# seceq/zkir

Hardware: AMD Instinct MI355X
Metric: trace rows/sec (2^20-cycle fib: execution-trace fill + BabyBear NTT/LDE + Poseidon2 Merkle commitment) (higher is better)
Workload: dtype u32 (Baby Bear, 31-bit modular) / u64 trace words

## Files before the change

zkir_amd/csrc/ntt.hip:

```cpp
#include <hip/hip_runtime.h>

#include <atomic>
#include <cstdlib>
#include <mutex>
#include <type_traits>

#include "../../include/zkir_amd.h"
#include "../../include/zkir_amd_experimental.h"
#include "babybear.h"
#include "host.h"

namespace {

constexpr int NT = 256;
__device__ __forceinline__ uint32_t bitrev(uint32_t x, int bits) { return bits == 0 ? 0u : __brev(x) >> (32 - bits); }

template <int K, int N, class F>
__device__ __forceinline__ void static_for(F&& f) {
  if constexpr (K < N) { f(std::integral_constant<int, K>{}); static_for<K + 1, N>(f); }
}

using u32x4 = uint32_t __attribute__((ext_vector_type(4)));
__device__ __forceinline__ u32x4 ld4(const uint4* p) { return *reinterpret_cast<const u32x4*>(p); }
__device__ __forceinline__ void st4(uint4* p, u32x4 v) { *reinterpret_cast<u32x4*>(p) = v; }

__device__ __forceinline__ void wave_sync_lds() { asm volatile("s_waitcnt lgkmcnt(0)" ::: "memory"); }

struct WTw { int32_t w, n; };
__device__ __forceinline__ WTw wtw(int32_t w) { return WTw{w, -w}; }
__device__ __forceinline__ void dit4w4(uint4& x0, uint4& x1, uint4& x2, uint4& x3, WTw w1, WTw w2, WTw w2i) {
#define ZKIR_Q(c, e) { int32_t a[4] = {(int32_t)x0.c, (int32_t)x1.c, (int32_t)x2.c, (int32_t)x3.c}, b[4] = {(int32_t)x0.e, (int32_t)x1.e, (int32_t)x2.e, (int32_t)x3.e}; \
                       bb::dit4w2(a, b, w1.w, w1.n, w2.w, w2.n, w2i.w, w2i.n); \
                       x0.c = (uint32_t)a[0]; x1.c = (uint32_t)a[1]; x2.c = (uint32_t)a[2]; x3.c = (uint32_t)a[3]; x0.e = (uint32_t)b[0]; x1.e = (uint32_t)b[1]; x2.e = (uint32_t)b[2]; x3.e = (uint32_t)b[3]; }
  ZKIR_Q(x, y) __builtin_amdgcn_sched_barrier(0); ZKIR_Q(z, w)
#undef ZKIR_Q
}
__device__ __forceinline__ void ct4w4(uint4& x0, uint4& x1, uint4& x2, uint4& x3, WTw w1, WTw w2, WTw w2i) { dit4w4(x0, x2, x1, x3, w1, w2, w2i); }
__device__ __forceinline__ void ct_twiddles(uint32_t sm, uint32_t f, bool unit, uint32_t j4_m, WTw& w1, WTw& w2, WTw& w2i) {
  uint32_t w2u;
  if (unit) { w2u = sm; w2 = wtw(bb::centre(sm)); }
  else { w2 = wtw(bb::mont_mul_centred(sm, f)); w2u = bb::wcanon(w2.w); }
  w1 = wtw(bb::mont_mul_centred(w2u, w2u)); w2i = wtw(bb::mont_mul_centred(w2u, j4_m));
}
__device__ __forceinline__ uint4 scale4(uint4 v, uint32_t g) {
  int32_t x[4] = {(int32_t)v.x, (int32_t)v.y, (int32_t)v.z, (int32_t)v.w};
  bb::wscale4(x, g);
  return make_uint4((uint32_t)x[0], (uint32_t)x[1], (uint32_t)x[2], (uint32_t)x[3]);
}
__device__ __forceinline__ void dit2w4(uint4& a, uint4& b, WTw w) {
#define ZKIR_Q(c) { int32_t p = (int32_t)a.c, q = (int32_t)b.c; bb::dit2w(p, q, w.w, w.n); a.c = (uint32_t)p; b.c = (uint32_t)q; }
  ZKIR_Q(x) ZKIR_Q(y) ZKIR_Q(z) ZKIR_Q(w)
#undef ZKIR_Q
}
__device__ __forceinline__ uint4 canon4(uint4 v) { return make_uint4(bb::wcanon((int32_t)v.x), bb::wcanon((int32_t)v.y), bb::wcanon((int32_t)v.z), bb::wcanon((int32_t)v.w)); }

template <bool DIT>
__global__ __launch_bounds__(NT) void ntt_stage_kernel(uint4* __restrict__ data, uint64_t blk_u4, int L, int s0, const uint32_t* __restrict__ tw, int canon) {
  uint4* x = data + (uint64_t)blockIdx.y * blk_u4;
  const uint64_t item = (uint64_t)blockIdx.x * NT + threadIdx.x;
  const uint32_t n = 1u << L;
  if (item >= (uint64_t)n) return;
  const uint32_t t = (uint32_t)(item >> 1), h = (uint32_t)(item & 1);
  uint32_t p, stride, w;
  if (DIT) { stride = 1u << s0; const uint32_t hi = t >> s0, lo = t & (stride - 1); p = (hi << (s0 + 1)) + lo; w = tw[lo << (L - s0 - 1)]; }
  else { stride = n >> (s0 + 1); const uint32_t hi = t / stride, lo = t % stride; p = hi * (n >> s0) + lo; w = tw[bitrev(hi, s0) << (L - s0 - 1)]; }
  uint4 a = x[(uint64_t)p * 2 + h], b = x[(uint64_t)(p + stride) * 2 + h];
  dit2w4(a, b, wtw(bb::centre(w)));
  if (DIT && canon) { a = canon4(a); b = canon4(b); }
  x[(uint64_t)p * 2 + h] = a; x[(uint64_t)(p + stride) * 2 + h] = b;
}

struct TraceSrc01 { zkir_trace_columns t; uint64_t n_real; };
__device__ __forceinline__ u32x4 trace_quad01(const TraceSrc01& q, uint32_t blk, uint32_t half, uint64_t i) {
  const bool pad = i >= q.n_real;
  const uint64_t src = pad ? q.n_real - 1 : i;
  u32x4 r;
  if (blk == 0 && half == 0) {
    const uint64_t pcv = q.t.pc[src];
    r.x = (uint32_t)((q.t.cycle[src] + (i - src)) % bb::P); r.y = (uint32_t)(pcv & 0xFFFFF); r.z = (uint32_t)((pcv >> 20) & 0xFFFFF); r.w = (uint32_t)(pcv >> 40);
  } else if (blk == 0) {
    const uint32_t w = q.t.instruction[src];
    r.x = w & 0x7F; r.y = (w >> 7) & 0xF; r.z = (w >> 11) & 0xF; r.w = (w >> 15) & 0xF;
  } else {
    auto limbs = [&](int g, uint32_t out[3]) {
      const uint64_t o = (uint64_t)g * q.t.reg_stride + src;
      const uint64_t v = q.t.registers[o];
      const int bits = q.t.reg_state[o] ? 30 : 20;
      const uint64_t mask = (1ull << bits) - 1;
      out[0] = (uint32_t)(v & mask); out[1] = (uint32_t)((v >> bits) & mask); out[2] = (uint32_t)(v >> (2 * bits));
    };
    uint32_t a[3], b[3];
    if (half == 0) { limbs(1, a); r.x = q.t.instruction[src] >> 19; r.y = a[0]; r.z = a[1]; r.w = a[2]; }
    else { limbs(2, a); limbs(3, b); r.x = a[0]; r.y = a[1]; r.z = a[2]; r.w = b[0]; }
  }
  return r;
}

template <bool DIT, int R, int C, int NTH, bool FUSED = false>
__global__ __launch_bounds__(NTH) void ntt_strided_r4_kernel(uint4* __restrict__ data, uint64_t blk_u4, uint32_t tiles_per_block, uint32_t total, int L, int s0,
                                                              const uint32_t* __restrict__ tw, const uint32_t* __restrict__ small, int log_small, uint32_t j4_m, int canon, TraceSrc01 fsrc = TraceSrc01{}) {
  constexpr int B = 2 * R;
  constexpr uint32_t POS = 1u << (B + C), QUADS = POS / 4, CMASK = (1u << C) - 1, PLANE = POS + 4;
  constexpr uint32_t MOVES = 2 * POS / NTH;
  static_assert(QUADS % NTH == 0 && NTH % (1 << C) == 0 && (2 * POS) % NTH == 0, "tile / thread geometry");
  extern __shared__ uint4 lds4[];
  const uint32_t n = 1u << L;
  const uint32_t stride_mid = DIT ? (1u << s0) : (n >> (s0 + B));
  const uint32_t lo_tiles = stride_mid >> C;
  auto geometry = [&](uint32_t w, uint4*& x, uint32_t& base, uint32_t& lo0, uint32_t& hi) {
    const uint32_t tile = w % tiles_per_block;
    x = data + (uint64_t)(w / tiles_per_block) * blk_u4;
    hi = tile / lo_tiles;
    lo0 = (tile % lo_tiles) << C;
    base = (DIT ? (hi << (s0 + B)) : hi * (n >> s0)) + lo0;
  };
  static_assert(QUADS == NTH, "one quad per lane and round");
  u32x4 pre[MOVES];
  uint4* x; uint32_t base, lo0, hi;
  uint32_t w = blockIdx.x;
  if (w >= total) return;
  uint32_t sm[R];
#pragma unroll
  for (int r = 0; r < R; r++) {
    const int b = 2 * r;
    const uint32_t qq = threadIdx.x >> C;
    if (!DIT) sm[r] = small[bitrev(qq >> (B - 2 - b), b) << (log_small - (b + 2))];
    else sm[r] = small[(qq & ((1u << b) - 1)) << (log_small - (b + 2))];
  }
  const bool unit = s0 == 0;
  uint32_t tf_next[R] = {};
  auto tile_factors = [&](uint32_t hi_t) {
    if (DIT || unit) return;
    const uint32_t e = bitrev(hi_t, s0);
#pragma unroll
    for (int r = 0; r < R; r++) tf_next[r] = tw[e << (L - s0 - 2 * r - 2)];
  };
  geometry(w, x, base, lo0, hi);
  static_for<0, (int)MOVES>([&](auto kc) {
    constexpr uint32_t k = decltype(kc)::value;
    const uint32_t e = threadIdx.x + k * NTH, row = e >> (C + 1), wv = e & ((2u << C) - 1);
    if constexpr (FUSED) pre[k] = trace_quad01(fsrc, w / tiles_per_block, wv & 1, (uint64_t)base + (uint64_t)row * stride_mid + (wv >> 1));
    else pre[k] = ld4(&x[((uint64_t)base + (uint64_t)row * stride_mid) * 2 + wv]);
  });
  uint32_t tw_cur = 0;
  if (DIT) tw_cur = tw[(lo0 + (threadIdx.x & CMASK)) << (L - s0 - B)];
  tile_factors(hi);
  for (;;) {
    static_for<0, (int)MOVES>([&](auto kc) {
      constexpr uint32_t k = decltype(kc)::value;
      const uint32_t e = threadIdx.x + k * NTH, row = e >> (C + 1), wv = e & ((2u << C) - 1);
      st4(&lds4[(wv & 1) * PLANE + ((row << C) | (wv >> 1))], pre[k]);
    });
    uint32_t tp[R];
    if (DIT) {
      uint32_t u = tw_cur;
#pragma unroll
      for (int r = R - 1; r >= 0; r--) { tp[r] = u; u = bb::mont_mul(u, u); u = bb::mont_mul(u, u); }
    } else {
#pragma unroll
      for (int r = 0; r < R; r++) tp[r] = tf_next[r];
    }
    __syncthreads();
    const uint32_t wn = w + gridDim.x;
    uint4* xn = x; uint32_t base_n = base, lo0_n = lo0, hi_n = hi;
    if (wn < total) {
      geometry(wn, xn, base_n, lo0_n, hi_n);
      static_for<0, (int)MOVES>([&](auto kc) {
        constexpr uint32_t k = decltype(kc)::value;
        const uint32_t e = threadIdx.x + k * NTH, row = e >> (C + 1), wv = e & ((2u << C) - 1);
        if constexpr (FUSED) pre[k] = trace_quad01(fsrc, wn / tiles_per_block, wv & 1, (uint64_t)base_n + (uint64_t)row * stride_mid + (wv >> 1));
        else pre[k] = ld4(&xn[((uint64_t)base_n + (uint64_t)row * stride_mid) * 2 + wv]);
      });
      if (DIT) tw_cur = tw[(lo0_n + (threadIdx.x & CMASK)) << (L - s0 - B)];
      tile_factors(hi_n);
    }
#pragma unroll
    for (int r = 0; r < R; r++) {
      const int b = 2 * r;
#pragma unroll
      for (uint32_t k = 0; k < QUADS / NTH; k++) {
        uint32_t q = threadIdx.x + k * NTH;
        asm volatile("" : "+v"(q));
        const uint32_t lo_l = q & CMASK, qq = q >> C;
        uint4* pl0 = lds4; uint4* pl1 = lds4 + PLANE;
        if constexpr (!DIT) {
          const int lg = B - 2 - b;
          const uint32_t h2 = 1u << lg, mid_lo = qq & (h2 - 1), mid_hi = qq >> lg;
          const uint32_t i0 = ((((mid_hi << (lg + 2)) | mid_lo)) << C) | lo_l, d = h2 << C;
          WTw w1, w2, w2i;
          ct_twiddles(sm[r], tp[r], unit, j4_m, w1, w2, w2i);
          uint4 x0 = pl0[i0], x1 = pl0[i0 + d], x2 = pl0[i0 + 2 * d], x3 = pl0[i0 + 3 * d];
          ct4w4(x0, x1, x2, x3, w1, w2, w2i);
          pl0[i0] = x0; pl0[i0 + d] = x1; pl0[i0 + 2 * d] = x2; pl0[i0 + 3 * d] = x3;
          __builtin_amdgcn_sched_barrier(0);
          uint4 y0 = pl1[i0], y1 = pl1[i0 + d], y2 = pl1[i0 + 2 * d], y3 = pl1[i0 + 3 * d];
          ct4w4(y0, y1, y2, y3, w1, w2, w2i);
          pl1[i0] = y0; pl1[i0 + d] = y1; pl1[i0 + 2 * d] = y2; pl1[i0 + 3 * d] = y3;
        } else {
          const uint32_t dm = 1u << b, mid_lo = qq & (dm - 1), mid_hi = qq >> b;
          const uint32_t i0 = ((((mid_hi << (b + 2)) | mid_lo)) << C) | lo_l, d = dm << C;
          const WTw w2 = wtw(bb::mont_mul_centred(tp[r], sm[r]));
          const uint32_t w2u = bb::wcanon(w2.w);
          const WTw w1 = wtw(bb::mont_mul_centred(w2u, w2u)), w2i = wtw(bb::mont_mul_centred(w2u, j4_m));
          uint4 x0 = pl0[i0], x1 = pl0[i0 + d], x2 = pl0[i0 + 2 * d], x3 = pl0[i0 + 3 * d];
          dit4w4(x0, x1, x2, x3, w1, w2, w2i);
          pl0[i0] = x0; pl0[i0 + d] = x1; pl0[i0 + 2 * d] = x2; pl0[i0 + 3 * d] = x3;
          __builtin_amdgcn_sched_barrier(0);
          uint4 y0 = pl1[i0], y1 = pl1[i0 + d], y2 = pl1[i0 + 2 * d], y3 = pl1[i0 + 3 * d];
          dit4w4(y0, y1, y2, y3, w1, w2, w2i);
          pl1[i0] = y0; pl1[i0 + d] = y1; pl1[i0 + 2 * d] = y2; pl1[i0 + 3 * d] = y3;
        }
      }
      const bool wave_local = !DIT ? (r + 1 < R && B - 2 - b <= 6 - C) : (r + 1 < R && b + 2 <= 6 - C);
      if (wave_local) wave_sync_lds(); else __syncthreads();
    }
#pragma unroll
    for (uint32_t k = 0; k < MOVES; k++) {
      const uint32_t e = threadIdx.x + k * NTH, row = e >> (C + 1), wv = e & ((2u << C) - 1);
      uint4 v = lds4[(wv & 1) * PLANE + ((row << C) | (wv >> 1))];
      if (DIT && canon) v = canon4(v);
      x[((uint64_t)base + (uint64_t)row * stride_mid) * 2 + wv] = v;
    }
    if (wn >= total) break;
    w = wn; x = xn; base = base_n; lo0 = lo0_n; hi = hi_n;
  }
}

template <bool DIT, int S>
__global__ __launch_bounds__(NT) void ntt_reg_kernel(uint4* __restrict__ data, uint64_t blk_u4, int L, int s0, const uint32_t* __restrict__ tw, uint32_t r4_m, uint32_t r8_m,
                                                       uint32_t r8_3_m, int canon) {
  constexpr int E = 1 << S;
  const uint32_t n = 1u << L;
  uint4* x = data + (uint64_t)blockIdx.y * blk_u4;
  const uint64_t item = (uint64_t)blockIdx.x * NT + threadIdx.x;
  if (item >= ((uint64_t)n >> S) * 2) return;
  const uint32_t t = (uint32_t)(item >> 1), h = (uint32_t)(item & 1);
  const uint32_t d = DIT ? (1u << s0) : (n >> (s0 + S));
  const uint32_t hi = t / d, lo = t % d;
  const uint64_t base = ((uint64_t)hi * d * E + lo) * 2 + h;
  uint4 v[E];
#pragma unroll
  for (int k = 0; k < E; k++) v[k] = x[base + (uint64_t)k * d * 2];
  if (!DIT) {
    const uint32_t Tf = tw[bitrev(hi, s0) << (L - s0 - S)];
    const uint32_t Tm = bb::mont_mul(Tf, Tf);
    if (S == 3) {
      const WTw t0 = wtw(bb::mont_mul_centred(Tm, Tm)), tm = wtw(bb::centre(Tm)), m1 = wtw(bb::mont_mul_centred(Tm, r4_m));
#pragma unroll
      for (int g = 0; g < 2; g++) ct4w4(v[g], v[g + 2], v[g + 4], v[g + 6], t0, tm, m1);
      const WTw wf[4] = {wtw(bb::centre(Tf)), wtw(bb::mont_mul_centred(Tf, r4_m)), wtw(bb::mont_mul_centred(Tf, r8_m)), wtw(bb::mont_mul_centred(Tf, r8_3_m))};
#pragma unroll
      for (int m = 0; m < 4; m++) dit2w4(v[2 * m], v[2 * m + 1], wf[m]);
    } else {
      ct4w4(v[0], v[1], v[2], v[3], wtw(bb::centre(Tm)), wtw(bb::centre(Tf)), wtw(bb::mont_mul_centred(Tf, r4_m)));
    }
  } else {
    const uint32_t Uf = tw[lo << (L - s0 - S)];
    const uint32_t Um = bb::mont_mul(Uf, Uf);
    if (S == 3) {
      const WTw u0 = wtw(bb::mont_mul_centred(Um, Um)), um = wtw(bb::centre(Um)), m1 = wtw(bb::mont_mul_centred(Um, r4_m));
#pragma unroll
      for (int g = 0; g < 8; g += 4) dit4w4(v[g], v[g + 1], v[g + 2], v[g + 3], u0, um, m1);
      const WTw wf[4] = {wtw(bb::centre(Uf)), wtw(bb::mont_mul_centred(Uf, r8_m)), wtw(bb::mont_mul_centred(Uf, r4_m)), wtw(bb::mont_mul_centred(Uf, r8_3_m))};
#pragma unroll
      for (int k = 0; k < 4; k++) dit2w4(v[k], v[k + 4], wf[k]);
    } else {
      dit4w4(v[0], v[1], v[2], v[3], wtw(bb::centre(Um)), wtw(bb::centre(Uf)), wtw(bb::mont_mul_centred(Uf, r4_m)));
    }
    if (canon) {
#pragma unroll
      for (int k = 0; k < E; k++) v[k] = canon4(v[k]);
    }
  }
#pragma unroll
  for (int k = 0; k < E; k++) x[base + (uint64_t)k * d * 2] = v[k];
}

inline unsigned cu_count() {
  static std::mutex mu;
  static unsigned cached[64] = {};
  int dev = 0;
  if (hipGetDevice(&dev) != hipSuccess || dev < 0 || dev >= 64) return 256u;
  std::lock_guard<std::mutex> lk(mu);
  if (!cached[dev]) { hipDeviceProp_t p; cached[dev] = hipGetDeviceProperties(&p, dev) == hipSuccess && p.multiProcessorCount > 0 ? (unsigned)p.multiProcessorCount : 256u; }
  return cached[dev];
}
inline int persist() { static const int v = getenv("ZKIR_NTT_PERSIST") ? atoi(getenv("ZKIR_NTT_PERSIST")) : 1; return v; }

template <bool DIT, int R, int C, int NTH, bool FUSED = false>
void launch_strided_r4(uint32_t* data, uint64_t n, uint32_t n_blocks, int L, int s0, const uint32_t* tw, const uint32_t* small, int log_small, uint32_t j4_m, hipStream_t s,
                       const TraceSrc01* fsrc = nullptr, int canon = 0) {
  constexpr size_t lds = 16u * 2 * ((1u << (2 * R + C)) + 4);
  auto k = ntt_strided_r4_kernel<DIT, R, C, NTH, FUSED>;
  static std::atomic<uint64_t> attr_done{0};
  int dev = 0; (void)hipGetDevice(&dev);
  const uint64_t bit = 1ull << (dev & 63);
  if (!(attr_done.load(std::memory_order_relaxed) & bit)) { (void)hipFuncSetAttribute(reinterpret_cast<const void*>(k), hipFuncAttributeMaxDynamicSharedMemorySize, (int)lds); attr_done.fetch_or(bit); }
  const uint32_t tiles = (uint32_t)(n >> (2 * R + C)), total = tiles * n_blocks;
  const unsigned per_cu = (unsigned)((160u << 10) / lds) > 0 ? (unsigned)((160u << 10) / lds) : 1u;
  unsigned grid = persist() ? cu_count() * (per_cu > 8 ? 8 : per_cu) : total;
  if (grid > total) grid = total;
  hipLaunchKernelGGL(k, dim3(grid), dim3(NTH), lds, s, (uint4*)data, 2 * n, tiles, total, L, s0, tw, small, log_small, j4_m, canon, fsrc ? *fsrc : TraceSrc01{});
}

inline int strided_c() { static const int c = getenv("ZKIR_NTT_C") ? atoi(getenv("ZKIR_NTT_C")) : 2; return c; }

template <bool DIT>
void run_strided_stages(uint32_t* data, uint64_t n, uint32_t n_blocks, int L, int s0, int stages, const uint32_t* tw, const uint32_t* small, int log_small, uint32_t j4_m,
                        uint32_t r8_m, uint32_t r8_3_m, hipStream_t s) {
  while (stages > 0) {
    int take;
    if (stages >= 10 && stages != 11) take = 10;
    else if (stages == 11) take = 8;
    else if (stages == 9) take = 6;
    else if (stages == 7) take = 4;
    else if (stages == 5) take = 3;
    else take = stages;
    const int canon = DIT && take == stages;
    switch (take) {
      case 10:
        if (strided_c() == 2) launch_strided_r4<DIT, 5, 2, 1024>(data, n, n_blocks, L, s0, tw, small, log_small, j4_m, s, nullptr, canon);
        else launch_strided_r4<DIT, 5, 1, 512>(data, n, n_blocks, L, s0, tw, small, log_small, j4_m, s, nullptr, canon);
        break;
      case 8: launch_strided_r4<DIT, 4, 3, 512>(data, n, n_blocks, L, s0, tw, small, log_small, j4_m, s, nullptr, canon); break;
      case 6: launch_strided_r4<DIT, 3, 4, 256>(data, n, n_blocks, L, s0, tw, small, log_small, j4_m, s, nullptr, canon); break;
      case 4: launch_strided_r4<DIT, 2, 5, 128>(data, n, n_blocks, L, s0, tw, small, log_small, j4_m, s, nullptr, canon); break;
      case 3:
        hipLaunchKernelGGL((ntt_reg_kernel<DIT, 3>), dim3((unsigned)(((n >> 3) * 2 + NT - 1) / NT), n_blocks), dim3(NT), 0, s, (uint4*)data, 2 * n, L, s0, tw, j4_m, r8_m, r8_3_m, canon);
        break;
      case 2:
        hipLaunchKernelGGL((ntt_reg_kernel<DIT, 2>), dim3((unsigned)(((n >> 2) * 2 + NT - 1) / NT), n_blocks), dim3(NT), 0, s, (uint4*)data, 2 * n, L, s0, tw, j4_m, r8_m, r8_3_m, canon);
        break;
      default:
        hipLaunchKernelGGL(ntt_stage_kernel<DIT>, dim3((unsigned)((n + NT - 1) / NT), n_blocks), dim3(NT), 0, s, (uint4*)data, 2 * n, L, s0, tw, canon);
        break;
    }
    s0 += take; stages -= take;
  }
}

__global__ __launch_bounds__(NT) void lde_small_kernel(const uint32_t* __restrict__ in, uint32_t* __restrict__ out, int L, const uint32_t* __restrict__ small_inv,
                                                        const uint32_t* __restrict__ small_fwd, const uint32_t* __restrict__ g_lo, const uint32_t* __restrict__ g_hi) {
  extern __shared__ uint32_t lds[];
  const uint32_t n = 1u << L;
  const uint32_t* x = in + (uint64_t)blockIdx.x * n * 8;
  uint32_t* y = out + (uint64_t)blockIdx.x * 2 * n * 8;
  for (int c = 0; c < 8; c++) {
    for (uint32_t e = threadIdx.x; e < n; e += NT) lds[e] = x[(uint64_t)e * 8 + c];
    __syncthreads();
    for (int b = 0; b < L; b++) {
      const int hb = L - 1 - b;
      const uint32_t half = 1u << hb;
      for (uint32_t q = threadIdx.x; q < (n >> 1); q += NT) {
        const uint32_t r_lo = q & (half - 1), r_hi = q >> hb;
        const uint32_t ia = (r_hi << (hb + 1)) | r_lo, ib = ia + half;
        const uint32_t a = lds[ia], bv = lds[ib];
        lds[ia] = bb::add(a, bv); lds[ib] = bb::mont_mul(bb::sub(a, bv), small_inv[r_lo << b]);
      }
      __syncthreads();
    }
    uint32_t v[2];
    int cnt = 0;
    for (uint32_t e = threadIdx.x; e < n; e += NT) { const uint32_t k = bitrev(e, L); v[cnt++] = bb::mont_mul(bb::mont_mul(lds[e], g_lo[k & 1023]), g_hi[k >> 10]); }
    __syncthreads();
    cnt = 0;
    for (uint32_t e = threadIdx.x; e < n; e += NT) { lds[2 * e] = v[cnt]; lds[2 * e + 1] = v[cnt]; cnt++; }
    __syncthreads();
    for (int s = 1; s <= L; s++) {
      const uint32_t half = 1u << s;
      for (uint32_t q = threadIdx.x; q < n; q += NT) {
        const uint32_t r_lo = q & (half - 1), r_hi = q >> s;
        const uint32_t ia = (r_hi << (s + 1)) | r_lo, ib = ia + half;
        const uint32_t a = lds[ia], t = bb::mont_mul(lds[ib], small_fwd[r_lo << (L - s)]);
        lds[ia] = bb::add(a, t); lds[ib] = bb::sub(a, t);
      }
      __syncthreads();
    }
    for (uint32_t e = threadIdx.x; e < 2 * n; e += NT) y[(uint64_t)e * 8 + c] = lds[e];
    __syncthreads();
  }
}

constexpr int MID_NT = 512;
__global__ __launch_bounds__(MID_NT) __attribute__((amdgpu_waves_per_eu(4, 4))) void lde_middle_r4_kernel(const uint4* __restrict__ in, uint4* __restrict__ out, uint32_t chunks_per_block, uint32_t total, int L,
                                                                const uint32_t* __restrict__ tw_inv, const uint32_t* __restrict__ small_inv, const uint32_t* __restrict__ small_fwd,
                                                                const uint32_t* __restrict__ g_lo, const uint32_t* __restrict__ g_hi, uint32_t j4_inv_m, uint32_t j4_fwd_m, int canon) {
  constexpr int Bm = 10;
  constexpr uint32_t APL = 1024;
  __shared__ uint4 A[2 * APL];
  __shared__ uint4 Bf[2048];
  const uint32_t n = 1u << L, t = threadIdx.x;
  uint32_t w = blockIdx.x;
  if (w >= total) return;
  uint32_t tw_i[5], tw_f[5];
#pragma unroll
  for (int r = 0; r < 5; r++) {
    const int lg = 8 - 2 * r;
    tw_i[r] = small_inv[bitrev((t & 255) >> lg, 2 * r) << lg];
    const int sft = 2 * r + 1;
    tw_f[r] = small_fwd[(t & ((1u << sft) - 1)) << (Bm - sft - 1)];
  }
  u32x4 pre[4];
  uint32_t cf_next[5];
  uint32_t glo[4], ghi[4];
  auto fetch = [&](uint32_t ww) {
    const uint4* x = in + ((uint64_t)(ww / chunks_per_block) * n + ((uint64_t)(ww % chunks_per_block) << Bm)) * 2;
#pragma unroll
    for (int k = 0; k < 4; k++) pre[k] = ld4(&x[t + k * MID_NT]);
    const uint32_t p0 = ((ww % chunks_per_block) << Bm) + 4 * (t & 255);
#pragma unroll
    for (int i = 0; i < 4; i++) { const uint32_t k = bitrev(p0 + i, L); glo[i] = g_lo[k & 1023]; ghi[i] = g_hi[k >> 10]; }
    const uint32_t ce = bitrev(ww % chunks_per_block, L - Bm);
#pragma unroll
    for (int r = 0; r < 5; r++) cf_next[r] = tw_inv[ce << (8 - 2 * r)];
  };
  fetch(w);
  for (;;) {
    const uint32_t base = (w % chunks_per_block) << Bm;
    uint4* y = out + (uint64_t)(w / chunks_per_block) * n * 4;
#pragma unroll
    for (int k = 0; k < 4; k++) { const uint32_t e = t + k * MID_NT; st4(&A[(e & 1) * APL + (e >> 1)], pre[k]); }
    uint32_t gs[4];
#pragma unroll
    for (int i = 0; i < 4; i++) gs[i] = bb::mont_mul(glo[i], ghi[i]);
    uint32_t cf[5];
#pragma unroll
    for (int r = 0; r < 5; r++) cf[r] = cf_next[r];
    __syncthreads();
    const uint32_t wn = w + gridDim.x;
    if (wn < total) fetch(wn);
    {
      const uint32_t q = t & 255;
      uint4* a = A + (t >> 8) * APL;
#pragma unroll
      for (int r = 0; r < 5; r++) {
        const int lg = 8 - 2 * r;
        const uint32_t h2 = 1u << lg, lo = q & (h2 - 1), hi = q >> lg;
        const uint32_t i0 = (hi << (lg + 2)) | lo;
        WTw c1, c2, c2i;
        ct_twiddles(tw_i[r], cf[r], false, j4_inv_m, c1, c2, c2i);
        uint4 x0 = a[i0], x1 = a[i0 + h2], x2 = a[i0 + 2 * h2], x3 = a[i0 + 3 * h2];
        ct4w4(x0, x1, x2, x3, c1, c2, c2i);
        if (r == 4) {
          x0 = scale4(x0, gs[0]); x1 = scale4(x1, gs[1]); x2 = scale4(x2, gs[2]); x3 = scale4(x3, gs[3]);
        }
        a[i0] = x0; a[i0 + h2] = x1; a[i0 + 2 * h2] = x2; a[i0 + 3 * h2] = x3;
        if (r >= 1 && r < 4) wave_sync_lds(); else __syncthreads();
      }
    }
#pragma unroll 1
    for (int h = 0; h < 2; h++) {
      const uint4* a = A + h * APL;
      uint4* F = h == 0 ? Bf : A;
#pragma unroll
      for (int r = 0; r < 5; r++) {
        const int s = 2 * r + 1;
        const uint32_t lo = t & ((1u << s) - 1), hi = t >> s;
        const uint32_t i0 = (hi << (s + 2)) | lo, d = 1u << s;
        const uint32_t w2 = tw_f[r];
        const WTw c2 = wtw(bb::centre(w2)), c1 = wtw(bb::mont_mul_centred(w2, w2)), c2i = wtw(bb::mont_mul_centred(w2, j4_fwd_m));
        uint4 x0, x1, x2, x3;
        if (r == 0) {
          x0 = a[i0 >> 1]; x1 = a[(i0 + d) >> 1]; x2 = a[(i0 + 2 * d) >> 1]; x3 = a[(i0 + 3 * d) >> 1];
          __syncthreads();
        } else { x0 = F[i0]; x1 = F[i0 + d]; x2 = F[i0 + 2 * d]; x3 = F[i0 + 3 * d]; }
        dit4w4(x0, x1, x2, x3, c1, c2, c2i);
        F[i0] = x0; F[i0 + d] = x1; F[i0 + 2 * d] = x2; F[i0 + 3 * d] = x3;
        if (r < 2) wave_sync_lds(); else __syncthreads();
      }
    }
#pragma unroll
    for (int k = 0; k < 4; k++) {
      const uint32_t e = t + k * MID_NT;
      uint4 v0 = Bf[e], v1 = A[e];
      if (canon) { v0 = canon4(v0); v1 = canon4(v1); }
      y[((uint64_t)2 * base + e) * 2] = v0; y[((uint64_t)2 * base + e) * 2 + 1] = v1;
    }
    __syncthreads();
    if (wn >= total) break;
    w = wn;
  }
}

}

namespace zkir {

void lde_run(const LdeTables& t, uint32_t* in, uint32_t n_blocks, uint32_t* out, void* stream) {
  hipStream_t s = (hipStream_t)stream;
  const int L = t.log_n;
  const uint32_t N = 1u << L;
  static const uint32_t j4_inv_m = bb::to_mont(bb::inv(bb::root_of_unity(2))), j4_fwd_m = bb::to_mont(bb::root_of_unity(2));
  static const uint32_t r8_fwd = bb::root_of_unity(3), r8_inv = bb::inv(r8_fwd);
  static const uint32_t r8_inv_m = bb::to_mont(r8_inv), r8_inv3_m = bb::to_mont(bb::mul(bb::mul(r8_inv, r8_inv), r8_inv));
  static const uint32_t r8_fwd_m = bb::to_mont(r8_fwd), r8_fwd3_m = bb::to_mont(bb::mul(bb::mul(r8_fwd, r8_fwd), r8_fwd));
  if (L < 10) {
    hipLaunchKernelGGL(lde_small_kernel, dim3(n_blocks), dim3(NT), (8u << L), s, in, out, L, t.small_inv, t.small_fwd, t.g_lo, t.g_hi);
    return;
  }
  run_strided_stages<false>(in, N, n_blocks, L, 0, L - 10, t.tw_inv, t.small_inv, 10, j4_inv_m, r8_inv_m, r8_inv3_m, s);
  {
    const uint32_t chunks = N >> 10, total = chunks * n_blocks;
    unsigned grid = persist() ? cu_count() * 2 : total;
    if (grid > total) grid = total;
    hipLaunchKernelGGL(lde_middle_r4_kernel, dim3(grid), dim3(MID_NT), 0, s, (const uint4*)in, (uint4*)out, chunks, total, L, t.tw_inv, t.small_inv, t.small_fwd, t.g_lo, t.g_hi,
                       j4_inv_m, j4_fwd_m, L == 10);
  }
  run_strided_stages<true>(out, (uint64_t)2 * N, n_blocks, L + 1, 11, L - 10, t.tw_fwd, t.small_fwd, 11, j4_fwd_m, r8_fwd_m, r8_fwd3_m, s);
}


bool strided_variant_run(const LdeTables& t, uint32_t* data, uint32_t n_blocks, int variant, bool dit, void* stream) {
  hipStream_t s = (hipStream_t)stream;
  const int L = dit ? t.log_n + 1 : t.log_n;
  if (t.log_n < 20) return false;
  const uint64_t n = (uint64_t)1 << L;
  static const uint32_t j4_inv_m = bb::to_mont(bb::inv(bb::root_of_unity(2))), j4_fwd_m = bb::to_mont(bb::root_of_unity(2));
  const uint32_t* tw = dit ? t.tw_fwd : t.tw_inv; const uint32_t* sm = dit ? t.small_fwd : t.small_inv;
  const int ls = dit ? 11 : 10; const uint32_t j4 = dit ? j4_fwd_m : j4_inv_m; const int s0 = dit ? 11 : 0;
#define ZKIR_VARIANT(R, C, NTH) do { if (dit) launch_strided_r4<true, R, C, NTH>(data, n, n_blocks, L, s0, tw, sm, ls, j4, s); else launch_strided_r4<false, R, C, NTH>(data, n, n_blocks, L, s0, tw, sm, ls, j4, s); } while (0)
  switch (variant) {
    case 0: ZKIR_VARIANT(5, 2, 1024); break;
    case 1: ZKIR_VARIANT(5, 1, 512); break;
    case 2: ZKIR_VARIANT(4, 3, 512); break;
    case 3: ZKIR_VARIANT(4, 2, 256); break;
    case 4: ZKIR_VARIANT(3, 4, 256); break;
    default: return false;
  }
#undef ZKIR_VARIANT
  return true;
}

bool lde_run_fused01(const LdeTables& t, const zkir_trace_columns* trace, uint64_t n_real, uint32_t* in, uint32_t n_blocks, uint32_t* out, void* stream) {
  hipStream_t s = (hipStream_t)stream;
  const int L = t.log_n;
  if (L < 20 || L == 21 || n_blocks < 3 || strided_c() != 2) return false;
  const uint32_t N = 1u << L;
  static const uint32_t j4_inv_m = bb::to_mont(bb::inv(bb::root_of_unity(2))), j4_fwd_m = bb::to_mont(bb::root_of_unity(2));
  static const uint32_t r8_fwd = bb::root_of_unity(3), r8_inv = bb::inv(r8_fwd);
  static const uint32_t r8_inv_m = bb::to_mont(r8_inv), r8_inv3_m = bb::to_mont(bb::mul(bb::mul(r8_inv, r8_inv), r8_inv));
  static const uint32_t r8_fwd_m = bb::to_mont(r8_fwd), r8_fwd3_m = bb::to_mont(bb::mul(bb::mul(r8_fwd, r8_fwd), r8_fwd));
  const TraceSrc01 src{*trace, n_real};
  launch_strided_r4<false, 5, 2, 1024, true>(in, N, 2, L, 0, t.tw_inv, t.small_inv, 10, j4_inv_m, s, &src);
  launch_strided_r4<false, 5, 2, 1024>(in + (uint64_t)2 * N * 8, N, n_blocks - 2, L, 0, t.tw_inv, t.small_inv, 10, j4_inv_m, s);
  if (L - 10 > 10) run_strided_stages<false>(in, N, n_blocks, L, 10, L - 20, t.tw_inv, t.small_inv, 10, j4_inv_m, r8_inv_m, r8_inv3_m, s);
  {
    const uint32_t chunks = N >> 10, total = chunks * n_blocks;
    unsigned grid = persist() ? cu_count() * 2 : total;
    if (grid > total) grid = total;
    hipLaunchKernelGGL(lde_middle_r4_kernel, dim3(grid), dim3(MID_NT), 0, s, (const uint4*)in, (uint4*)out, chunks, total, L, t.tw_inv, t.small_inv, t.small_fwd, t.g_lo, t.g_hi,
                       j4_inv_m, j4_fwd_m, L == 10);
  }
  run_strided_stages<true>(out, (uint64_t)2 * N, n_blocks, L + 1, 11, L - 10, t.tw_fwd, t.small_fwd, 11, j4_fwd_m, r8_fwd_m, r8_fwd3_m, s);
  return true;
}

}
```

Baseline: 192.4 million.

## Fuse first inverse stage into register load and interleave forward halves in LDE mid kernel

The first inverse radix-4 stage now runs on the prefetched registers before they are written to LDS, which removes one LDS round trip and one barrier. The two forward NTT halves are interleaved inside a single stage loop, so each stage syncs once for both halves instead of once per half. The last forward stage stores straight to global memory, dropping the LDS readback and the trailing copy loop. Scheduling barriers and the changed sync placement make LDS hazards across loop iterations more delicate to get right.

```diff
diff --git a/zkir_amd/csrc/ntt.hip b/zkir_amd/csrc/ntt.hip
--- a/zkir_amd/csrc/ntt.hip
+++ b/zkir_amd/csrc/ntt.hip
@@ -418,14 +418,21 @@
   for (;;) {
     const uint32_t base = (w % chunks_per_block) << Bm;
     uint4* y = out + (uint64_t)(w / chunks_per_block) * n * 4;
-#pragma unroll
-    for (int k = 0; k < 4; k++) { const uint32_t e = t + k * MID_NT; st4(&A[(e & 1) * APL + (e >> 1)], pre[k]); }
     uint32_t gs[4];
 #pragma unroll
     for (int i = 0; i < 4; i++) gs[i] = bb::mont_mul(glo[i], ghi[i]);
     uint32_t cf[5];
 #pragma unroll
     for (int r = 0; r < 5; r++) cf[r] = cf_next[r];
+    {
+      WTw c1, c2, c2i;
+      ct_twiddles(tw_i[0], cf[0], false, j4_inv_m, c1, c2, c2i);
+      uint4 x0 = make_uint4(pre[0].x, pre[0].y, pre[0].z, pre[0].w), x1 = make_uint4(pre[1].x, pre[1].y, pre[1].z, pre[1].w);
+      uint4 x2 = make_uint4(pre[2].x, pre[2].y, pre[2].z, pre[2].w), x3 = make_uint4(pre[3].x, pre[3].y, pre[3].z, pre[3].w);
+      ct4w4(x0, x1, x2, x3, c1, c2, c2i);
+      uint4* a = A + (t & 1) * APL + (t >> 1);
+      a[0] = x0; a[256] = x1; a[512] = x2; a[768] = x3;
+    }
     __syncthreads();
     const uint32_t wn = w + gridDim.x;
     if (wn < total) fetch(wn);
@@ -433,7 +440,7 @@
       const uint32_t q = t & 255;
       uint4* a = A + (t >> 8) * APL;
 #pragma unroll
-      for (int r = 0; r < 5; r++) {
+      for (int r = 1; r < 5; r++) {
         const int lg = 8 - 2 * r;
         const uint32_t h2 = 1u << lg, lo = q & (h2 - 1), hi = q >> lg;
         const uint32_t i0 = (hi << (lg + 2)) | lo;
@@ -448,36 +455,45 @@
         if (r >= 1 && r < 4) wave_sync_lds(); else __syncthreads();
       }
     }
-#pragma unroll 1
-    for (int h = 0; h < 2; h++) {
-      const uint4* a = A + h * APL;
-      uint4* F = h == 0 ? Bf : A;
-#pragma unroll
-      for (int r = 0; r < 5; r++) {
-        const int s = 2 * r + 1;
-        const uint32_t lo = t & ((1u << s) - 1), hi = t >> s;
-        const uint32_t i0 = (hi << (s + 2)) | lo, d = 1u << s;
-        const uint32_t w2 = tw_f[r];
-        const WTw c2 = wtw(bb::centre(w2)), c1 = wtw(bb::mont_mul_centred(w2, w2)), c2i = wtw(bb::mont_mul_centred(w2, j4_fwd_m));
-        uint4 x0, x1, x2, x3;
-        if (r == 0) {
-          x0 = a[i0 >> 1]; x1 = a[(i0 + d) >> 1]; x2 = a[(i0 + 2 * d) >> 1]; x3 = a[(i0 + 3 * d) >> 1];
-          __syncthreads();
-        } else { x0 = F[i0]; x1 = F[i0 + d]; x2 = F[i0 + 2 * d]; x3 = F[i0 + 3 * d]; }
+#pragma unroll
+    for (int r = 0; r < 5; r++) {
+      const int s = 2 * r + 1;
+      const uint32_t lo = t & ((1u << s) - 1), hi = t >> s;
+      const uint32_t i0 = (hi << (s + 2)) | lo, d = 1u << s;
+      const uint32_t w2 = tw_f[r];
+      const WTw c2 = wtw(bb::centre(w2)), c1 = wtw(bb::mont_mul_centred(w2, w2)), c2i = wtw(bb::mont_mul_centred(w2, j4_fwd_m));
+      uint4 x0, x1, x2, x3, z0, z1, z2, z3;
+      if (r == 0) {
+        x0 = A[i0 >> 1]; x1 = A[(i0 + d) >> 1]; x2 = A[(i0 + 2 * d) >> 1]; x3 = A[(i0 + 3 * d) >> 1];
         dit4w4(x0, x1, x2, x3, c1, c2, c2i);
-        F[i0] = x0; F[i0 + d] = x1; F[i0 + 2 * d] = x2; F[i0 + 3 * d] = x3;
-        if (r < 2) wave_sync_lds(); else __syncthreads();
+        Bf[i0] = x0; Bf[i0 + d] = x1; Bf[i0 + 2 * d] = x2; Bf[i0 + 3 * d] = x3;
+        __builtin_amdgcn_sched_barrier(0);
+        z0 = A[APL + (i0 >> 1)]; z1 = A[APL + ((i0 + d) >> 1)]; z2 = A[APL + ((i0 + 2 * d) >> 1)]; z3 = A[APL + ((i0 + 3 * d) >> 1)];
+        __syncthreads();
+        dit4w4(z0, z1, z2, z3, c1, c2, c2i);
+        A[i0] = z0; A[i0 + d] = z1; A[i0 + 2 * d] = z2; A[i0 + 3 * d] = z3;
+      } else {
+        x0 = Bf[i0]; x1 = Bf[i0 + d]; x2 = Bf[i0 + 2 * d]; x3 = Bf[i0 + 3 * d];
+        dit4w4(x0, x1, x2, x3, c1, c2, c2i);
+        uint4* o = y + ((uint64_t)2 * base + t) * 2;
+        if (r < 4) { Bf[i0] = x0; Bf[i0 + d] = x1; Bf[i0 + 2 * d] = x2; Bf[i0 + 3 * d] = x3; }
+        else {
+          if (canon) { x0 = canon4(x0); x1 = canon4(x1); x2 = canon4(x2); x3 = canon4(x3); }
+          o[0] = x0; o[2 * MID_NT] = x1; o[4 * MID_NT] = x2; o[6 * MID_NT] = x3;
+        }
+        __builtin_amdgcn_sched_barrier(0);
+        z0 = A[i0]; z1 = A[i0 + d]; z2 = A[i0 + 2 * d]; z3 = A[i0 + 3 * d];
+        dit4w4(z0, z1, z2, z3, c1, c2, c2i);
+        if (r < 4) { A[i0] = z0; A[i0 + d] = z1; A[i0 + 2 * d] = z2; A[i0 + 3 * d] = z3; }
+        else {
+          if (canon) { z0 = canon4(z0); z1 = canon4(z1); z2 = canon4(z2); z3 = canon4(z3); }
+          o[1] = z0; o[2 * MID_NT + 1] = z1; o[4 * MID_NT + 1] = z2; o[6 * MID_NT + 1] = z3;
+        }
       }
-    }
-#pragma unroll
-    for (int k = 0; k < 4; k++) {
-      const uint32_t e = t + k * MID_NT;
-      uint4 v0 = Bf[e], v1 = A[e];
-      if (canon) { v0 = canon4(v0); v1 = canon4(v1); }
-      y[((uint64_t)2 * base + e) * 2] = v0; y[((uint64_t)2 * base + e) * 2 + 1] = v1;
-    }
-    __syncthreads();
+      if (r < 2) wave_sync_lds(); else if (r < 4) __syncthreads();
+    }
     if (wn >= total) break;
+    __syncthreads();
     w = wn;
   }
 }
```

After: 194.2 million (median of 6 runs). Within noise of the previous version (+1.0%).
